# matteosantama/dantzig

Hardware: AMD Instinct MI355X
Metric: simplex_iterations_per_sec (higher is better)
Workload: dtype f64

## Files before the change

dantzig_amd/csrc/k_price.hip:

```cpp
#include "k_price_kernels.h"

static_assert(DZG_RL_WORK_SLOTS == DZG_PRICE_CSC_BLOCKS, "work counters of k_price_csc_rl");

static int resolve(int kernel)
{
    return kernel == DZG_PRICE_WAVE || kernel == DZG_PRICE_TREE ? kernel : DZG_PRICE_SEQ;
}

#define PRICE_ARGS ctl, A, lda, m, q, plist, nonbasis, var_col, v, dz, z, zbar, rz_r, rz_k, rz_h, col0

static void launch_tree(int ncols, const DzgCtl *ctl, const double *A, long long lda, int m, int q,
                        const int *plist, const int *nonbasis, const int *var_col, const double *v,
                        double *dz, const double *z, const double *zbar, double *rz_r, int *rz_k,
                        double *rz_h, int col0, const int *pcode, hipStream_t st, int rows_T = 0,
                        int need_kind = -1)
{
    const dim3 grid(DZG_PRICE_TREE_BLOCKS), block(256);
    const int per_wave = (ncols + 4 * DZG_PRICE_TREE_BLOCKS - 1) / (4 * DZG_PRICE_TREE_BLOCKS);
    const int passes = (per_wave + 15) / 16;
    const int cw = passes > 0 ? (per_wave + passes - 1) / passes : 1;
#define TREE(CW, DEPTH, TP)                                                                          \
    hipLaunchKernelGGL((k_price_tree<CW, DEPTH, TP>), grid, block, 0, st, PRICE_ARGS, pcode, rows_T, need_kind)
    if (per_wave == 15 || per_wave == 16) { TREE(8, 2, 2); return; }
    switch (cw) {
    case 16: TREE(16, 2, 1); break;
    case 15: TREE(15, 2, 1); break;
    case 14: TREE(14, 2, 1); break;
    case 13: TREE(13, 2, 1); break;
    case 12: TREE(12, 3, 1); break;
    case 11: TREE(11, 3, 1); break;
    case 10: TREE(10, 2, 2); break;
    case 9: TREE(9, 2, 2); break;
    case 8: TREE(8, 2, 2); break;
    case 7: TREE(7, 4, 1); break;
    case 6: TREE(6, 3, 2); break;
    case 5: TREE(5, 4, 2); break;
    case 4: TREE(4, 8, 1); break;
    case 3: TREE(3, 10, 1); break;
    case 2: TREE(2, 16, 1); break;
    default: TREE(1, 32, 1); break;
    }
#undef TREE
}

static void launch(int kernel, int ncols, const DzgCtl *ctl, const double *A, long long lda, int m, int q,
                   const int *plist, const int *nonbasis, const int *var_col, const double *v,
                   double *dz, const double *z, const double *zbar, double *rz_r, int *rz_k,
                   double *rz_h, int col0, const int *pcode, hipStream_t st, int rows_T = 0,
                   int need_kind = -1)
{
    if (q <= 0) return;
    if (resolve(kernel) == DZG_PRICE_TREE)
        launch_tree(ncols, PRICE_ARGS, pcode, st, rows_T, need_kind);
    else if (resolve(kernel) == DZG_PRICE_WAVE)
        hipLaunchKernelGGL((k_price_wave2<4>), dim3(DZG_PRICE_WAVE_BLOCKS), dim3(256), 0, st, ctl, A,
                           lda, m, q, plist, nonbasis, var_col, v, dz, z, zbar, rz_r, rz_k, rz_h, col0);
    else
        hipLaunchKernelGGL((k_price_seq2<16>), dim3(DZG_PRICE_SEQ_BLOCKS), dim3(256), 0, st, ctl, A,
                           lda, m, q, plist, nonbasis, var_col, v, dz, z, zbar, rz_r, rz_k, rz_h, col0);
}

int dzg_price_partials(int kernel)
{
    if (kernel == DZG_PRICE_CSC_KERNEL) return DZG_PRICE_CSC_BLOCKS;
    if (resolve(kernel) == DZG_PRICE_TREE) return DZG_PRICE_TREE_BLOCKS;
    return resolve(kernel) == DZG_PRICE_WAVE ? DZG_PRICE_WAVE_BLOCKS : DZG_PRICE_SEQ_BLOCKS;
}

static int rl_grid(void)
{
    static const int g = [] {
        const char *e = std::getenv("DZG_RL_GRID");
        const int v = e ? std::atoi(e) : 1024;
        return v < 1 ? 1 : (v > DZG_PRICE_CSC_BLOCKS ? DZG_PRICE_CSC_BLOCKS : v);
    }();
    return g;
}

int dzg_price_partials_dev(const DzgDev &d, int kernel)
{
    if (!d.csc) return dzg_price_partials(kernel);
    if (d.spb && d.lcnt && kernel != DZG_PRICE_SEQ) return rl_grid();
    return DZG_PRICE_CSC_BLOCKS;
}

static void launch_csc(const DzgDev &d, const int *plist, const double *z, const double *zbar,
                       double *rz_r, int *rz_k, double *rz_h, bool seq_order, hipStream_t st)
{
    if (d.q <= 0) return;
    if (z && !seq_order)
        hipLaunchKernelGGL(k_price_csc_tree, dim3(DZG_PRICE_CSC_BLOCKS), dim3(256), 0, st, d.ctl,
                           d.cptr, d.ridx, d.cval, d.q, plist, d.nbcode, (const int *)nullptr, d.v,
                           d.dz, z, zbar, rz_r, rz_k, rz_h, d.col0, plist ? d.pcode : (const int *)nullptr);
    else
        hipLaunchKernelGGL(k_price_csc, dim3(DZG_PRICE_CSC_BLOCKS), dim3(256), 0, st, d.ctl, d.cptr,
                           d.ridx, d.cval, d.q, plist, d.nonbasis, d.var_col, d.v, d.dz, z, zbar,
                           rz_r, rz_k, rz_h, d.col0);
}

void dzg_launch_price(const DzgDev &d, int kernel, hipStream_t st)
{
    if (d.csc) {
        launch_csc(d, nullptr, nullptr, nullptr, nullptr, nullptr, nullptr, true, st);
        return;
    }
    launch(kernel, d.q, d.ctl, d.A, d.lda, d.m, d.q, nullptr, d.nonbasis, d.var_col, d.v, d.dz, nullptr,
           nullptr, nullptr, nullptr, nullptr, 0, nullptr, st);
}

void dzg_launch_transpose_to_rows(const double *A, long long lda, int m, int n, double *At,
                                  long long ldt, hipStream_t st)
{
    if (m <= 0 || ldt <= 0) return;
    hipLaunchKernelGGL(k_transpose_to_rows, dim3((unsigned)((ldt + 31) / 32), (unsigned)((m + 31) / 32)),
                       dim3(32, 8), 0, st, A, lda, m, n, At, ldt);
}
int dzg_price_rows_groups(void) { return PR_GMAX; }

static int price_small_k(void)
{
    static const int v = [] {
        const char *e = std::getenv("DZG_PRICE_SMALL_K");
        const int x = e ? std::atoi(e) : 480;
        return x < 0 ? 0 : (x > PRS_ROWS - 1 ? PRS_ROWS - 1 : x);
    }();
    return v;
}
int dzg_price_small(const DzgDev &d, int kernel)
{
    return d.cpos && d.vc && d.world <= 1 && !d.rs && dzg_price_rows_certain(d, kernel) && d.k_hint < price_small_k() &&
           (d.ldt + PRS_TILE - 1) / PRS_TILE <= 4096;
}
int dzg_price_small_partials(const DzgDev &d) { return (int)((d.ldt + PRS_TILE - 1) / PRS_TILE); }

int dzg_price_rows_certain(const DzgDev &d, int kernel)
{
    return !d.csc && d.At && d.q > 0 && resolve(kernel) == DZG_PRICE_TREE && d.k_hint > 0 &&
           d.k_hint < d.rows_T && d.k_hint < d.fold_k;
}

void dzg_launch_price_fast(const DzgDev &d, int kernel, hipStream_t st, int need_kind, int skip_finish,
                           int small, unsigned long long *dbg)
{
    if (small) {
        if (d.k_hint < 8 * DZG_PR_BATCH - 1)
            hipLaunchKernelGGL(k_price_rows_small<false>, dim3(dzg_price_small_partials(d)), dim3(512), 0, st,
                               d.ctl, d.rows_T, d.At, d.ldt, d.col1 - d.col0, d.drow, d.vc, d.cpos, d.q,
                               d.nbcode, d.v, d.dz, d.z, d.zbar, d.rz_r, d.rz_k, d.rz_h, dbg);
        else
            hipLaunchKernelGGL(k_price_rows_small<true>, dim3(dzg_price_small_partials(d)), dim3(512), 0, st,
                               d.ctl, d.rows_T, d.At, d.ldt, d.col1 - d.col0, d.drow, d.vc, d.cpos, d.q,
                               d.nbcode, d.v, d.dz, d.z, d.zbar, d.rz_r, d.rz_k, d.rz_h, dbg);
        return;
    }
    if (d.csc) {
        if (d.spb && d.lcnt && kernel != DZG_PRICE_SEQ) {
            if (d.q > 0)
                hipLaunchKernelGGL(k_price_csc_rl, dim3(rl_grid()), dim3(256), 0, st, d.ctl,
                                   d.cptr, d.lcnt, d.lent, d.q, d.plist, d.pcode, d.nbcode, d.v,
                                   d.dz, d.z, d.zbar, d.rz_r, d.rz_k, d.rz_h, d.rl_work);
            return;
        }
        launch_csc(d, d.plist, d.z, d.zbar, d.rz_r, d.rz_k, d.rz_h, kernel == DZG_PRICE_SEQ, st);
        return;
    }
    int ncols = d.col1 - d.col0;
    if (d.price_cols_hint > 0 && d.price_cols_hint < ncols) ncols = d.price_cols_hint;
    int rows_T = 0;
    if (d.At && d.q > 0 && resolve(kernel) == DZG_PRICE_TREE) {
        rows_T = d.rows_T;
        const bool rows_possible = d.k_lo_hint < 0 || d.k_lo_hint < rows_T;
        const bool cols_possible = d.k_hint <= 0 || d.k_hint >= rows_T;
        const int rows_rule = cols_possible ? rows_T : 0x7fffffff;
        if (!rows_possible) rows_T = 0;
        if (rows_possible) {
            hipLaunchKernelGGL((k_price_rows<2>), dim3((unsigned)((d.ldt + 511) / 512), PR_GMAX),
                               dim3(256), 0, st, d.ctl, rows_rule, d.At, d.ldt, d.drow, d.bcode, d.vc,
                               d.ppart, need_kind);
            if (!(skip_finish && !cols_possible))
                hipLaunchKernelGGL(k_price_rows_finish, dim3(DZG_PRICE_TREE_BLOCKS), dim3(256), 0, st,
                                   d.ctl, rows_rule, d.ppart, d.ldt, d.q, d.plist, d.pcode, d.nbcode, d.bcode,
                                   d.col0, d.v, d.dz, d.z, d.zbar, d.rz_r, d.rz_k, d.rz_h, PR_GMAX, need_kind);
        }
        if (!cols_possible) return;
    }
    launch(kernel, ncols, d.ctl, d.A, d.lda, d.m, d.q, d.plist, d.nbcode, nullptr, d.v, d.dz, d.z,
           d.zbar, d.rz_r, d.rz_k, d.rz_h, d.col0, d.pcode, st, rows_T, need_kind);
}

void dzg_launch_price_raw(int kernel, int m, long long lda, const double *A, const int *cols,
                          int ncols, const double *v, double *out, hipStream_t st)
{
    launch(kernel, ncols, nullptr, A, lda, m, ncols, nullptr, cols, nullptr, v, out, nullptr, nullptr,
           nullptr, nullptr, nullptr, 0, nullptr, st);
}

void dzg_launch_price_csc_raw(const long long *cptr, const int *ridx, const double *cval,
                              const int *cols, int ncols, const double *v, double *out,
                              hipStream_t st)
{
    if (ncols <= 0) return;
    hipLaunchKernelGGL(k_price_csc, dim3(DZG_PRICE_CSC_BLOCKS), dim3(256), 0, st,
                       (const DzgCtl *)nullptr, cptr, ridx, cval, ncols, (const int *)nullptr, cols,
                       (const int *)nullptr, v, out, (const double *)nullptr,
                       (const double *)nullptr, (double *)nullptr, (int *)nullptr,
                       (double *)nullptr, 0);
}
```

dantzig_amd/csrc/k_price_kernels.h:

```cpp
#pragma once
#include "common.h"

typedef double double2_t __attribute__((ext_vector_type(2)));

__device__ __forceinline__ int price_code(const int *__restrict__ nonbasis,
                                          const int *__restrict__ var_col, int pos)
{
    const int v = nonbasis[pos];
    return var_col ? var_col[v] : v;
}

__device__ __forceinline__ void price_candidate(DzgCand2 &best, double dzk, int pos, double mu,
                                                double tau, const double *__restrict__ z,
                                                const double *__restrict__ zbar)
{
    const double zk = z[pos], scaled = mu * zbar[pos];
    const double den = zk + scaled;
    DzgCand2 c;
    c.r = dzg_div(dzk, den);
    c.k = pos;
    c.h = -__builtin_inf();
    if (c.r > 0.0) best = dzg_better2(best, c);
    if (dzg_noise_zero(den, zk, scaled, tau)) best.h = __builtin_inf();
}

__device__ __forceinline__ void price_candidate_v(DzgCand2 &best, double dzk, int pos, double mu,
                                                  double tau, double zk, double zbk)
{
    const double scaled = mu * zbk;
    const double den = zk + scaled;
    DzgCand2 c;
    c.r = dzg_div(dzk, den);
    c.k = pos;
    c.h = -__builtin_inf();
    if (c.r > 0.0) best = dzg_better2(best, c);
    if (dzg_noise_zero(den, zk, scaled, tau)) best.h = __builtin_inf();
}

__device__ __forceinline__ void price_slack_positions(DzgCand2 &best, int q,
                                                      const int *__restrict__ nonbasis,
                                                      const int *__restrict__ var_col,
                                                      const double *__restrict__ v,
                                                      double *__restrict__ dz, double mu,
                                                      double tau, const double *__restrict__ z,
                                                      const double *__restrict__ zbar)
{
    const int nthreads = gridDim.x * blockDim.x;
    for (int pos = blockIdx.x * blockDim.x + threadIdx.x; pos < q; pos += nthreads) {
        const int code = price_code(nonbasis, var_col, pos);
        if (code < 0) {
            const double p = 1.0 * -v[-1 - code];
            const double d = 0.0 + p;
            dz[pos] = d;
            if (z) price_candidate(best, d, pos, mu, tau, z, zbar);
        }
    }
}

__device__ __forceinline__ void price_publish(DzgCand2 best, double *__restrict__ rz_r,
                                              int *__restrict__ rz_k, double *__restrict__ rz_h)
{
    best = dzg_block_best2(best);
    if (rz_r && threadIdx.x == 0) {
        rz_r[blockIdx.x] = best.r;
        rz_k[blockIdx.x] = best.k;
        rz_h[blockIdx.x] = best.h;
    }
}

__device__ __forceinline__ void price_publish_small(DzgCand2 best, double *__restrict__ rz_r,
                                                    int *__restrict__ rz_k, double *__restrict__ rz_h)
{
    best = dzg_block_best2_flat<8>(best, false);
    if (rz_r && threadIdx.x == 0) {
        rz_r[blockIdx.x] = best.r;
        rz_k[blockIdx.x] = best.k;
        rz_h[blockIdx.x] = best.h;
    }
}

template <int CW, int DEPTH = 2, int DBG = 0, bool NT = true>
__global__ __launch_bounds__(256) void k_price_seq2(
    const DzgCtl *ctl, const double *__restrict__ A, long long lda, int m, int q,
    const int *__restrict__ plist, const int *__restrict__ nonbasis,
    const int *__restrict__ var_col, const double *__restrict__ v, double *__restrict__ dz,
    const double *__restrict__ z, const double *__restrict__ zbar, double *__restrict__ rz_r,
    int *__restrict__ rz_k, double *__restrict__ rz_h, int col0 = 0)
{
    constexpr int TR = 128, PAD = 2;
    __shared__ __attribute__((aligned(16))) double tile[4][CW][TR + PAD];
    if (ctl && ctl->status != DZG_RUNNING) return;
    const int lane = threadIdx.x & 63, wave = threadIdx.x >> 6;
    const int nw = gridDim.x * 4;
    const int wg = blockIdx.x * 4 + wave;
    const double mu = ctl ? ctl->mu : 0.0, tau = ctl ? ctl->tau : 0.0;
    DzgCand2 best = dzg_cand2_none();
    price_slack_positions(best, q, nonbasis, var_col, v, dz, mu, tau, z, zbar);

    const int count = plist ? (int)ctl->nb_struct : q;
    const int base = count / nw, rem = count % nw;
    const int start = wg * base + (wg < rem ? wg : rem);
    const int cnt = base + (wg < rem ? 1 : 0);
    const int ntiles = (m + TR - 1) / TR;
    double(*mytile)[TR + PAD] = tile[wave];

    for (int c0 = 0; c0 < cnt; c0 += CW) {
        const int nc = (cnt - c0) < CW ? (cnt - c0) : CW;
        int mypos = -1, mycode = -1;
        if (lane < nc) {
            const int idx = start + c0 + lane;
            mypos = plist ? plist[idx] : idx;
            mycode = price_code(nonbasis, var_col, mypos);
        }
        int lastcode = col0;
#pragma unroll
        for (int l = 0; l < CW; ++l) {
            const int code_l = __builtin_amdgcn_readlane(mycode, l);
            if (code_l >= 0) lastcode = code_l;
        }
        long long off[CW];
#pragma unroll
        for (int l = 0; l < CW; ++l) {
            const int code_l = __builtin_amdgcn_readlane(mycode, l);
            off[l] = (long long)((code_l >= 0 ? code_l : lastcode) - col0) * lda;
        }
        double2_t rg[DEPTH][CW], vg[DEPTH];
        double dbg_sink = 0.0;
        long long cyc_park = 0, cyc_fetch = 0, cyc_walk = 0;
        const int lastpair = (int)lda - 2;
        const int lastv = ((m + 1) & ~1) - 2 >= 0 ? ((m + 1) & ~1) - 2 : 0;

        auto fetch = [&](int t, double2_t(&reg)[CW], double2_t &vreg) {
            const int row = t * TR + 2 * lane;
            const int rowc = row < lda ? row : lastpair;
#pragma unroll
            for (int l = 0; l < CW; ++l) {
                const double2_t *gp = reinterpret_cast<const double2_t *>(A + off[l] + rowc);
                reg[l] = NT ? __builtin_nontemporal_load(gp) : *gp;
            }
            vreg = *reinterpret_cast<const double2_t *>(v + (row < m ? row : lastv));
        };
        auto park = [&](int t, const double2_t(&reg)[CW], const double2_t &vreg) {
            if (DBG == 2) {
#pragma unroll
                for (int l = 0; l < CW; ++l) dbg_sink += reg[l].x + reg[l].y;
                return;
            }
            const int row = t * TR + 2 * lane;
            const bool inside = row < lda && row < m + 1;
            const double nv0 = -vreg.x, nv1 = -vreg.y;
            const double2_t zero = {0.0, 0.0};
            __builtin_amdgcn_wave_barrier();
#pragma unroll
            for (int l = 0; l < CW; ++l) {
                double2_t pr;
                pr.x = reg[l].x != 0.0 ? reg[l].x * nv0 : 0.0;
                pr.y = reg[l].y != 0.0 ? reg[l].y * nv1 : 0.0;
                *reinterpret_cast<double2_t *>(&mytile[l][2 * lane]) = inside ? pr : zero;
            }
            __builtin_amdgcn_fence(__ATOMIC_RELEASE, "wavefront");
            __builtin_amdgcn_wave_barrier();
        };
        double acc = 0.0;
        const double *colp = mytile[lane & (CW - 1)];
        auto walk = [&](int t) {
            if (DBG != 0 && DBG != 4) return;
            const int row0 = t * TR;
            const int rows = (m - row0) < TR ? (m - row0) : TR;
            if (lane < CW) {
                if (rows == TR) {
                    double2_t buf[2][8];
#pragma unroll
                    for (int j = 0; j < 8; ++j)
                        buf[0][j] = *reinterpret_cast<const double2_t *>(colp + 2 * j);
#pragma unroll
                    for (int c = 0; c < TR / 16; ++c) {
                        if (c + 1 < TR / 16) {
#pragma unroll
                            for (int j = 0; j < 8; ++j)
                                buf[(c + 1) & 1][j] = *reinterpret_cast<const double2_t *>(
                                    colp + 16 * (c + 1) + 2 * j);
                        }
#pragma unroll
                        for (int j = 0; j < 8; ++j) {
                            acc = acc + buf[c & 1][j].x;
                            acc = acc + buf[c & 1][j].y;
                        }
                    }
                } else {
                    for (int r = 0; r < rows; ++r) acc = acc + colp[r];
                }
            }
        };

#pragma unroll
        for (int d = 0; d < DEPTH; ++d) fetch(d < ntiles ? d : ntiles - 1, rg[d], vg[d]);
        int t = 0;
        for (; t + 2 * DEPTH - 1 < ntiles; t += DEPTH) {
#pragma unroll
            for (int d = 0; d < DEPTH; ++d) {
                if (DBG == 4) {
                    const long long s0 = __builtin_amdgcn_s_memtime();
                    park(t + d, rg[d], vg[d]);
                    __builtin_amdgcn_s_waitcnt(0xC07F);
                    const long long s1 = __builtin_amdgcn_s_memtime();
                    fetch(t + DEPTH + d, rg[d], vg[d]);
                    const long long s2 = __builtin_amdgcn_s_memtime();
                    walk(t + d);
                    asm volatile("" ::"v"(acc));
                    const long long s3 = __builtin_amdgcn_s_memtime();
                    cyc_park += s1 - s0;
                    cyc_fetch += s2 - s1;
                    cyc_walk += s3 - s2;
                } else {
                    park(t + d, rg[d], vg[d]);
                    fetch(t + DEPTH + d, rg[d], vg[d]);
                    walk(t + d);
                }
            }
        }
#pragma unroll
        for (int d = 0; d < DEPTH; ++d) {
            if (t + d < ntiles) {
                park(t + d, rg[d], vg[d]);
                if (t + DEPTH + d < ntiles) fetch(t + DEPTH + d, rg[d], vg[d]);
                walk(t + d);
            }
        }
#pragma unroll
        for (int d = 0; d < DEPTH; ++d) {
            if (t + DEPTH + d < ntiles) {
                park(t + DEPTH + d, rg[d], vg[d]);
                walk(t + DEPTH + d);
            }
        }
        if (DBG != 0 && DBG != 4) acc = dbg_sink + mytile[lane & (CW - 1)][lane];
        if (DBG == 4 && lane == 0) {
            dz[q + 3 * wg + 0] = (double)cyc_park;
            dz[q + 3 * wg + 1] = (double)cyc_fetch;
            dz[q + 3 * wg + 2] = (double)cyc_walk;
        }
        if (lane < nc && mycode >= 0) {
            dz[mypos] = acc;
            if (z) price_candidate(best, acc, mypos, mu, tau, z, zbar);
        }
    }
    price_publish(best, rz_r, rz_k, rz_h);
}

template <int U>
__global__ __launch_bounds__(256) void k_price_wave2(
    const DzgCtl *ctl, const double *__restrict__ A, long long lda, int m, int q,
    const int *__restrict__ plist, const int *__restrict__ nonbasis,
    const int *__restrict__ var_col, const double *__restrict__ v, double *__restrict__ dz,
    const double *__restrict__ z, const double *__restrict__ zbar, double *__restrict__ rz_r,
    int *__restrict__ rz_k, double *__restrict__ rz_h, int col0 = 0)
{
    if (ctl && ctl->status != DZG_RUNNING) return;
    const int lane = threadIdx.x & 63;
    const int wg = (blockIdx.x * blockDim.x + threadIdx.x) >> 6;
    const int nw = (gridDim.x * blockDim.x) >> 6;
    const double mu = ctl ? ctl->mu : 0.0, tau = ctl ? ctl->tau : 0.0;
    DzgCand2 best = dzg_cand2_none();
    price_slack_positions(best, q, nonbasis, var_col, v, dz, mu, tau, z, zbar);
    const int count = plist ? (int)ctl->nb_struct : q;
    const int mpad = (m + 1) & ~1;
    for (int idx = wg; idx < count; idx += nw) {
        const int pos = plist ? plist[idx] : idx;
        const int code = price_code(nonbasis, var_col, pos);
        if (code < 0) continue;
        const double *col = A + (long long)(code - col0) * lda;
        double acc[U];
#pragma unroll
        for (int u = 0; u < U; ++u) acc[u] = 0.0;
        int r = 2 * lane;
        for (; r + 128 * (U - 1) < mpad; r += 128 * U) {
            double2_t c[U], w[U];
#pragma unroll
            for (int u = 0; u < U; ++u)
                c[u] = __builtin_nontemporal_load(
                    reinterpret_cast<const double2_t *>(col + r + 128 * u));
#pragma unroll
            for (int u = 0; u < U; ++u) w[u] = *reinterpret_cast<const double2_t *>(v + r + 128 * u);
#pragma unroll
            for (int u = 0; u < U; ++u) {
                acc[u] = fma(c[u].x, w[u].x, acc[u]);
                acc[u] = fma(c[u].y, w[u].y, acc[u]);
            }
        }
        for (; r < mpad; r += 128) {
            const double2_t c0 = *reinterpret_cast<const double2_t *>(col + r);
            const double2_t w0 = *reinterpret_cast<const double2_t *>(v + r);
            acc[0] = fma(c0.x, w0.x, acc[0]);
            acc[0] = fma(c0.y, w0.y, acc[0]);
        }
        double s = 0.0;
#pragma unroll
        for (int u = 0; u < U; ++u) s += acc[u];
#pragma unroll
        for (int off = 32; off > 0; off >>= 1) s += __shfl_xor(s, off, DZG_WAVE);
        if (lane == 0) {
            dz[pos] = -s;
            if (z) price_candidate(best, -s, pos, mu, tau, z, zbar);
        }
    }
    price_publish(best, rz_r, rz_k, rz_h);
}

template <int CW, int DEPTH, int TP = 1>
__global__ __launch_bounds__(256) void k_price_tree(
    const DzgCtl *ctl, const double *__restrict__ A, long long lda, int m, int q,
    const int *__restrict__ plist, const int *__restrict__ nonbasis,
    const int *__restrict__ var_col, const double *__restrict__ v, double *__restrict__ dz,
    const double *__restrict__ z, const double *__restrict__ zbar, double *__restrict__ rz_r,
    int *__restrict__ rz_k, double *__restrict__ rz_h, int col0 = 0,
    const int *__restrict__ pcode = nullptr, int rows_T = 0, int need_kind = -1)
{
    constexpr int TR = 128;
    if (ctl && ctl->status != DZG_RUNNING) return;
    if (rows_T > 0 && ctl->ncompact < rows_T) return;
    if (need_kind >= 0 && ctl->kind != need_kind) return;
    const int lane = threadIdx.x & 63, wave = threadIdx.x >> 6;
    const int nw = gridDim.x * 4;
    const int wg = blockIdx.x * 4 + wave;
    const double mu = ctl ? ctl->mu : 0.0, tau = ctl ? ctl->tau : 0.0;
    DzgCand2 best = dzg_cand2_none();
    const int nthreads = gridDim.x * blockDim.x;
    const int spos = blockIdx.x * blockDim.x + threadIdx.x;
    int scode = 0;
    if (spos < q) scode = price_code(nonbasis, var_col, spos);
    double sv = 0.0, sz = 0.0, szb = 0.0;
    bool slack_loaded = false;

    const int count = plist ? (int)ctl->nb_struct : q;
    const int base = count / nw, rem = count % nw;
    const int start = wg * base + (wg < rem ? wg : rem);
    const int cnt = base + (wg < rem ? 1 : 0);
    const int ntiles = (m + TR - 1) / TR;
    const int ngroups = (ntiles + TP - 1) / TP;
    const int lastpair = (int)lda - 2;
    const int lastv = ((m + 1) & ~1) - 2 >= 0 ? ((m + 1) & ~1) - 2 : 0;

    for (int c0 = 0; c0 < cnt; c0 += CW) {
        const int nc = (cnt - c0) < CW ? (cnt - c0) : CW;
        int mypos = -1, mycode = -1;
        if (lane < nc) {
            const int idx = start + c0 + lane;
            mypos = plist ? plist[idx] : idx;
            mycode = pcode ? pcode[idx] : price_code(nonbasis, var_col, mypos);
        }
        int lastcode = col0;
#pragma unroll
        for (int l = 0; l < CW; ++l) {
            const int code_l = __builtin_amdgcn_readlane(mycode, l);
            if (code_l >= 0) lastcode = code_l;
        }
        long long off[CW];
#pragma unroll
        for (int l = 0; l < CW; ++l) {
            const int code_l = __builtin_amdgcn_readlane(mycode, l);
            off[l] = (long long)((code_l >= 0 ? code_l : lastcode) - col0) * lda;
        }
        double2_t rg[DEPTH][TP][CW], vg[DEPTH][TP];
        double acc[CW];
#pragma unroll
        for (int l = 0; l < CW; ++l) acc[l] = 0.0;
        double zc = 0.0, zbc = 0.0;
        if (z && lane < nc && mycode >= 0) {
            zc = z[mypos];
            zbc = zbar[mypos];
        }
        if (!slack_loaded) {
            slack_loaded = true;
            if (scode < 0) {
                sv = v[-1 - scode];
                if (z) {
                    sz = z[spos];
                    szb = zbar[spos];
                }
            }
        }

        auto fetch = [&](int g, double2_t(&reg)[TP][CW], double2_t(&vreg)[TP]) {
#pragma unroll
            for (int l = 0; l < CW; ++l)
#pragma unroll
                for (int u = 0; u < TP; ++u) {
                    const int row = (g * TP + u) * TR + 2 * lane;
                    const int rowc = row < lda ? row : lastpair;
                    reg[u][l] = __builtin_nontemporal_load(
                        reinterpret_cast<const double2_t *>(A + off[l] + rowc));
                }
#pragma unroll
            for (int u = 0; u < TP; ++u) {
                const int row = (g * TP + u) * TR + 2 * lane;
                vreg[u] = *reinterpret_cast<const double2_t *>(v + (row < m ? row : lastv));
            }
        };
        auto consume = [&](int g, const double2_t(&reg)[TP][CW], const double2_t(&vreg)[TP]) {
#pragma unroll
            for (int u = 0; u < TP; ++u) {
                const bool inside = (g * TP + u) * TR + 2 * lane < m;
#pragma unroll
                for (int l = 0; l < CW; ++l) {
                    const double ax = inside ? reg[u][l].x : 0.0, ay = inside ? reg[u][l].y : 0.0;
                    acc[l] = fma(ax, vreg[u].x, acc[l]);
                    acc[l] = fma(ay, vreg[u].y, acc[l]);
                }
            }
        };
#pragma unroll
        for (int d = 0; d < DEPTH; ++d) fetch(d < ngroups ? d : ngroups - 1, rg[d], vg[d]);
        int t = 0;
        for (; t + 2 * DEPTH - 1 < ngroups; t += DEPTH) {
#pragma unroll
            for (int d = 0; d < DEPTH; ++d) {
                consume(t + d, rg[d], vg[d]);
                fetch(t + DEPTH + d, rg[d], vg[d]);
            }
        }
#pragma unroll
        for (int d = 0; d < DEPTH; ++d) {
            if (t + d < ngroups) {
                consume(t + d, rg[d], vg[d]);
                if (t + DEPTH + d < ngroups) fetch(t + DEPTH + d, rg[d], vg[d]);
            }
        }
#pragma unroll
        for (int d = 0; d < DEPTH; ++d)
            if (t + DEPTH + d < ngroups) consume(t + DEPTH + d, rg[d], vg[d]);
        double mine = 0.0;
#pragma unroll
        for (int l = 0; l < CW; ++l) {
            double s = acc[l];
#pragma unroll
            for (int o = 32; o > 0; o >>= 1) s += __shfl_xor(s, o, DZG_WAVE);
            if (lane == l) mine = s;
        }
        if (lane < nc && mycode >= 0) {
            dz[mypos] = -mine;
            if (z) price_candidate_v(best, -mine, mypos, mu, tau, zc, zbc);
        }
    }
    if (scode < 0) {
        if (!slack_loaded) {
            sv = v[-1 - scode];
            if (z) {
                sz = z[spos];
                szb = zbar[spos];
            }
        }
        const double p = 1.0 * -sv;
        const double d = 0.0 + p;
        dz[spos] = d;
        if (z) price_candidate_v(best, d, spos, mu, tau, sz, szb);
    }
    for (int pos = spos + nthreads; pos < q; pos += nthreads) {
        const int code = price_code(nonbasis, var_col, pos);
        if (code < 0) {
            const double p = 1.0 * -v[-1 - code];
            const double d = 0.0 + p;
            dz[pos] = d;
            if (z) price_candidate(best, d, pos, mu, tau, z, zbar);
        }
    }
    price_publish(best, rz_r, rz_k, rz_h);
}

__global__ __launch_bounds__(256) void k_price_csc(
    const DzgCtl *ctl, const long long *__restrict__ cptr, const int *__restrict__ ridx,
    const double *__restrict__ cval, int q, const int *__restrict__ plist,
    const int *__restrict__ nonbasis, const int *__restrict__ var_col,
    const double *__restrict__ v, double *__restrict__ dz, const double *__restrict__ z,
    const double *__restrict__ zbar, double *__restrict__ rz_r, int *__restrict__ rz_k,
    double *__restrict__ rz_h, int col0)
{
    if (ctl && ctl->status != DZG_RUNNING) return;
    const double mu = ctl ? ctl->mu : 0.0, tau = ctl ? ctl->tau : 0.0;
    DzgCand2 best = dzg_cand2_none();
    price_slack_positions(best, q, nonbasis, var_col, v, dz, mu, tau, z, zbar);
    const int count = plist ? (int)ctl->nb_struct : q;
    const int lane = threadIdx.x & 63, sub = lane & 7, gbase = lane & ~7;
    const int group = (blockIdx.x * blockDim.x + threadIdx.x) >> 3;
    const int ngroups = (gridDim.x * blockDim.x) >> 3;
    for (int idx0 = 0; idx0 < count; idx0 += ngroups) {
        const int idx = idx0 + group;
        int pos = -1, code = -1;
        long long e0 = 0, e1 = 0;
        if (idx < count) {
            pos = plist ? plist[idx] : idx;
            code = price_code(nonbasis, var_col, pos);
            if (code >= 0) {
                e0 = cptr[code - col0];
                e1 = cptr[code - col0 + 1];
            }
        }
        long long span = e1 - e0;
#pragma unroll
        for (int off = 32; off >= 8; off >>= 1) {
            const long long o = __shfl_xor(span, off, DZG_WAVE);
            span = o > span ? o : span;
        }
        double acc = 0.0;
        for (long long base = 0; base < span; base += 8) {
            const long long e = e0 + base + sub;
            double p = 0.0;
            if (e < e1) p = cval[e] * -v[ridx[e]];
#pragma unroll
            for (int t = 0; t < 8; ++t) {
                const double pt = __shfl(p, gbase + t, DZG_WAVE);
                if (e0 + base + t < e1) acc = acc + pt;
            }
        }
        if (code >= 0 && sub == 0) {
            dz[pos] = acc;
            if (z) price_candidate(best, acc, pos, mu, tau, z, zbar);
        }
    }
    price_publish(best, rz_r, rz_k, rz_h);
}

__global__ __launch_bounds__(256) void k_price_csc_tree(
    const DzgCtl *ctl, const long long *__restrict__ cptr, const int *__restrict__ ridx,
    const double *__restrict__ cval, int q, const int *__restrict__ plist,
    const int *__restrict__ nonbasis, const int *__restrict__ var_col,
    const double *__restrict__ v, double *__restrict__ dz, const double *__restrict__ z,
    const double *__restrict__ zbar, double *__restrict__ rz_r, int *__restrict__ rz_k,
    double *__restrict__ rz_h, int col0, const int *__restrict__ pcode = nullptr)
{
    if (ctl && ctl->status != DZG_RUNNING) return;
    const double mu = ctl ? ctl->mu : 0.0, tau = ctl ? ctl->tau : 0.0;
    DzgCand2 best = dzg_cand2_none();
    const int nthreads = gridDim.x * blockDim.x;
    const int spos = blockIdx.x * blockDim.x + threadIdx.x;
    int scode = 0;
    if (spos < q) scode = price_code(nonbasis, var_col, spos);
    double sv = 0.0, sz = 0.0, szb = 0.0;
    bool slack_loaded = false;
    const int count = plist ? (int)ctl->nb_struct : q;
    const int sub = threadIdx.x & 7;
    const int group = (blockIdx.x * blockDim.x + threadIdx.x) >> 3;
    const int ngroups = (gridDim.x * blockDim.x) >> 3;
    for (int idx0 = 0; idx0 < count; idx0 += ngroups) {
        const int idx = idx0 + group;
        int pos = -1, code = -1;
        long long e0 = 0, e1 = 0;
        if (idx < count) {
            pos = plist ? plist[idx] : idx;
            code = pcode ? pcode[idx] : price_code(nonbasis, var_col, pos);
            if (code >= 0) {
                e0 = cptr[code - col0];
                e1 = cptr[code - col0 + 1];
            }
        }
        double zc = 0.0, zbc = 0.0;
        if (z && code >= 0 && sub == 0) {
            zc = z[pos];
            zbc = zbar[pos];
        }
        if (!slack_loaded) {
            slack_loaded = true;
            if (scode < 0) {
                sv = v[-1 - scode];
                if (z) {
                    sz = z[spos];
                    szb = zbar[spos];
                }
            }
        }
        double a0 = 0.0, a1 = 0.0;
        long long e = e0 + sub;
        for (; e + 8 < e1; e += 16) {
            const int r0 = ridx[e], r1 = ridx[e + 8];
            const double c0 = cval[e], c1 = cval[e + 8];
            a0 = fma(c0, v[r0], a0);
            a1 = fma(c1, v[r1], a1);
        }
        if (e < e1) a0 = fma(cval[e], v[ridx[e]], a0);
        double acc = a0 + a1;
#pragma unroll
        for (int off = 4; off > 0; off >>= 1) acc += __shfl_xor(acc, off, DZG_WAVE);
        if (code >= 0 && sub == 0) {
            dz[pos] = -acc;
            if (z) price_candidate_v(best, -acc, pos, mu, tau, zc, zbc);
        }
    }
    if (scode < 0) {
        if (!slack_loaded) {
            sv = v[-1 - scode];
            if (z) {
                sz = z[spos];
                szb = zbar[spos];
            }
        }
        const double p = 1.0 * -sv;
        const double d = 0.0 + p;
        dz[spos] = d;
        if (z) price_candidate_v(best, d, spos, mu, tau, sz, szb);
    }
    for (int pos = spos + nthreads; pos < q; pos += nthreads) {
        const int code = price_code(nonbasis, var_col, pos);
        if (code < 0) {
            const double p = 1.0 * -v[-1 - code];
            const double d = 0.0 + p;
            dz[pos] = d;
            if (z) price_candidate(best, d, pos, mu, tau, z, zbar);
        }
    }
    price_publish(best, rz_r, rz_k, rz_h);
}

#define RL_LPC 4
__global__ __launch_bounds__(256) void k_price_csc_rl(
    const DzgCtl *ctl, const long long *__restrict__ cptr, const int *__restrict__ lcnt,
    const DzgLiveEntry *__restrict__ lent, int q,
    const int *__restrict__ plist, const int *__restrict__ pcode, const int *__restrict__ nbcode,
    const double *__restrict__ v, double *__restrict__ dz, const double *__restrict__ z,
    const double *__restrict__ zbar, double *__restrict__ rz_r, int *__restrict__ rz_k,
    double *__restrict__ rz_h, unsigned long long *__restrict__ work)
{
    __shared__ unsigned int s_work[4];
    const int nthreads = gridDim.x * blockDim.x;
    const int spos = blockIdx.x * blockDim.x + threadIdx.x;
    const int sub = threadIdx.x & (RL_LPC - 1);
    const int group = spos / RL_LPC;
    const int ngroups = nthreads / RL_LPC;
    int scode = 0, pos0 = -1, code0 = -1;
    if (spos < q) scode = nbcode[spos];
    if (group < q) {
        pos0 = plist[group];
        code0 = pcode[group];
    }
    const int status = ctl->status, count = (int)ctl->nb_struct;
    const double mu = ctl->mu, tau = ctl->tau;
    if (status != DZG_RUNNING) return;
    DzgCand2 best = dzg_cand2_none();
    double sv = 0.0, sz = 0.0, szb = 0.0;
    if (scode < 0) {
        sv = v[-1 - scode];
        sz = z[spos];
        szb = zbar[spos];
    }
    unsigned int walked = 0;
    for (int idx0 = 0; idx0 < count; idx0 += ngroups) {
        const int idx = idx0 + group;
        int pos = -1, code = -1;
        long long e0 = 0, e1 = 0;
        if (idx < count) {
            pos = idx0 == 0 ? pos0 : plist[idx];
            code = idx0 == 0 ? code0 : pcode[idx];
            if (code >= 0) {
                e0 = cptr[code];
                e1 = e0 + lcnt[code];
            }
        }
        double zc = 0.0, zbc = 0.0;
        if (code >= 0 && sub == 0) {
            zc = z[pos];
            zbc = zbar[pos];
            walked += (unsigned int)(e1 - e0);
        }
        double a0 = 0.0, a1 = 0.0;
        long long e = e0 + sub;
        for (; e + RL_LPC < e1; e += 2 * RL_LPC) {
            const DzgLiveEntry n0 = lent[e], n1 = lent[e + RL_LPC];
            a0 = fma(n0.val, v[n0.row], a0);
            a1 = fma(n1.val, v[n1.row], a1);
        }
        if (e < e1) {
            const DzgLiveEntry n0 = lent[e];
            a0 = fma(n0.val, v[n0.row], a0);
        }
        double acc = a0 + a1;
#pragma unroll
        for (int off = RL_LPC / 2; off > 0; off >>= 1) acc += __shfl_xor(acc, off, DZG_WAVE);
        if (code >= 0 && sub == 0) {
            dz[pos] = -acc;
            price_candidate_v(best, -acc, pos, mu, tau, zc, zbc);
        }
    }
    if (scode < 0) {
        const double p = 1.0 * -sv;
        const double d = 0.0 + p;
        dz[spos] = d;
        price_candidate_v(best, d, spos, mu, tau, sz, szb);
    }
    for (int pos = spos + nthreads; pos < q; pos += nthreads) {
        const int code = nbcode[pos];
        if (code < 0) {
            const double p = 1.0 * -v[-1 - code];
            const double d = 0.0 + p;
            dz[pos] = d;
            price_candidate(best, d, pos, mu, tau, z, zbar);
        }
    }
#pragma unroll
    for (int off = 32; off > 0; off >>= 1) walked += __shfl_xor(walked, off, DZG_WAVE);
    if ((threadIdx.x & 63) == 0) s_work[threadIdx.x >> 6] = walked;
    price_publish(best, rz_r, rz_k, rz_h);
    if (threadIdx.x == 0)
        __hip_atomic_fetch_add(work + blockIdx.x,
                               (unsigned long long)s_work[0] + s_work[1] + s_work[2] + s_work[3],
                               __ATOMIC_RELAXED, __HIP_MEMORY_SCOPE_AGENT);
}

#define PR_GMAX DZG_PR_GMAX
#define PR_BATCH DZG_PR_BATCH
#define PR_PIPE 8
template <int VEC, int PIPE = PR_PIPE>
__global__ __launch_bounds__(256) void k_price_rows(
    const DzgCtl *ctl, int rows_T, const double *__restrict__ At, long long ldt,
    const int *__restrict__ drow, const int *__restrict__ bcode, const double *__restrict__ vc,
    double *__restrict__ part, int need_kind = -1)
{
    typedef double vec_t __attribute__((ext_vector_type(2)));
    __shared__ long long s_off[256];
    __shared__ double s_coef[256];
    const int status = ctl->status, k = ctl->ncompact, lp = ctl->leave_pos;
    if (status != DZG_RUNNING || k >= rows_T) return;
    if (need_kind >= 0 && ctl->kind != need_kind) return;
    int G = (k + 1 + PR_BATCH - 1) / PR_BATCH;
    G = G > (int)gridDim.y ? (int)gridDim.y : G;
    const int g = blockIdx.y;
    if (g >= G) return;
    const int lcode = lp >= 0 ? bcode[lp] : 0;
    const int nrows = k + (lcode < 0 ? 1 : 0);
    const long long j0 = ((long long)blockIdx.x * 256 + threadIdx.x) * VEC;
    const bool live = j0 < ldt;
    const double *col = At + (live ? j0 : 0);
    double acc[VEC];
#pragma unroll
    for (int e = 0; e < VEC; ++e) acc[e] = 0.0;
    for (int cbase = g; cbase < nrows; cbase += 256 * G) {
        __syncthreads();
        const int c = cbase + (int)threadIdx.x * G;
        if (c < nrows) {
            const int row = c < k ? drow[c] : -1 - lcode;
            s_off[threadIdx.x] = (long long)row * ldt;
            s_coef[threadIdx.x] = c < k ? vc[c] : 1.0;
        }
        __syncthreads();
        const int left = (nrows - cbase + G - 1) / G;
        const int n = left < 256 ? left : 256;
        const int bfull = n / PIPE;
        vec_t ra[PIPE][VEC / 2], rb[PIPE][VEC / 2];
#define PR_LOAD(B, REG)                                                                              \
    _Pragma("unroll") for (int u = 0; u < PIPE; ++u) {                                            \
        const double *src = col + s_off[(B) * PIPE + u];                                          \
        _Pragma("unroll") for (int h = 0; h < VEC / 2; ++h)                                          \
            REG[u][h] = __builtin_nontemporal_load(reinterpret_cast<const vec_t *>(src) + h);        \
    }
#define PR_FMA(B, REG)                                                                               \
    _Pragma("unroll") for (int u = 0; u < PIPE; ++u) {                                            \
        const double cf = s_coef[(B) * PIPE + u];                                                 \
        _Pragma("unroll") for (int h = 0; h < VEC / 2; ++h) {                                        \
            acc[2 * h] = fma(cf, REG[u][h].x, acc[2 * h]);                                           \
            acc[2 * h + 1] = fma(cf, REG[u][h].y, acc[2 * h + 1]);                                   \
        }                                                                                            \
    }
        int bi = 0;
        if (bfull > 0) { PR_LOAD(0, ra) }
        while (bi + 2 < bfull) {
            PR_LOAD(bi + 1, rb)
            PR_FMA(bi, ra)
            PR_LOAD(bi + 2, ra)
            PR_FMA(bi + 1, rb)
            bi += 2;
        }
        if (bfull - bi == 2) {
            PR_LOAD(bi + 1, rb)
            PR_FMA(bi, ra)
            PR_FMA(bi + 1, rb)
        } else if (bfull - bi == 1) {
            PR_FMA(bi, ra)
        }
#undef PR_LOAD
#undef PR_FMA
        {
            const int i0 = bfull * PIPE;
#pragma unroll
            for (int u = 0; u < PIPE; ++u)
                if (i0 + u < n) {
                    const double *src = col + s_off[i0 + u];
#pragma unroll
                    for (int h = 0; h < VEC / 2; ++h)
                        ra[u][h] = __builtin_nontemporal_load(reinterpret_cast<const vec_t *>(src) + h);
                }
#pragma unroll
            for (int u = 0; u < PIPE; ++u)
                if (i0 + u < n) {
                    const double cf = s_coef[i0 + u];
#pragma unroll
                    for (int h = 0; h < VEC / 2; ++h) {
                        acc[2 * h] = fma(cf, ra[u][h].x, acc[2 * h]);
                        acc[2 * h + 1] = fma(cf, ra[u][h].y, acc[2 * h + 1]);
                    }
                }
        }
    }
    if (live) {
        double *dst = part + (long long)g * ldt + j0;
#pragma unroll
        for (int e = 0; e < VEC; ++e) dst[e] = acc[e];
    }
}

#define PRS_TILE 64
#define PRS_ROWS 512
#define PRS_STAMP_SLOT 4
template <bool WIDE>
__global__ __launch_bounds__(512) void k_price_rows_small(
    const DzgCtl *__restrict__ ctl, int rows_T, const double *__restrict__ At, long long ldt, int ncols,
    const int *__restrict__ drow, const double *__restrict__ vc,
    const int *__restrict__ cpos, int q, const int *__restrict__ nbcode, const double *__restrict__ v,
    double *__restrict__ dz, const double *__restrict__ z, const double *__restrict__ zbar,
    double *__restrict__ rz_r, int *__restrict__ rz_k, double *__restrict__ rz_h,
    unsigned long long *dbg)
{
    __shared__ long long s_off[PRS_ROWS];
    __shared__ double s_coef[PRS_ROWS];
    __shared__ double s_part[PR_GMAX][PRS_TILE];
    ChainStamps ts;
    ts.start(dbg);
    const int tid = threadIdx.x, lane = tid & 63, wave = tid >> 6;
    const int spos = blockIdx.x * 512 + tid;
    int scode = 0;
    if (spos < q) scode = nbcode[spos];
    const long long j = (long long)blockIdx.x * PRS_TILE + lane;
    int pos = -1;
    if (wave == 0 && j < ncols) pos = cpos[j];
    const int status = ctl->status, k = ctl->ncompact, lp = ctl->leave_pos;
    const int lcode_c = ctl->leave_code;
    const double mu = ctl->mu, tau = ctl->tau;
    asm volatile("" ::"s"(status), "s"(k), "s"(lp), "s"(lcode_c), "s"(mu), "s"(tau));
    if (status != DZG_RUNNING || k >= rows_T || k >= PRS_ROWS) return;
    ts.mark(PRS_STAMP_SLOT);
    const int lcode = lp >= 0 ? lcode_c : 0;
    if (tid < k) {
        s_off[tid] = (long long)drow[tid] * ldt;
        s_coef[tid] = vc[tid];
    }
    double sv = 0.0, sz = 0.0, szb = 0.0, zc = 0.0, zbc = 0.0;
    if (scode < 0) {
        sv = v[-1 - scode];
        sz = z[spos];
        szb = zbar[spos];
    }
    if (pos >= 0) {
        zc = z[pos];
        zbc = zbar[pos];
    }
    const int nrows = k + (lcode < 0 ? 1 : 0);
    if (tid == k && lcode < 0) {
        s_off[k] = (long long)(-1 - lcode) * ldt;
        s_coef[k] = 1.0;
    }
    int G = (k + 1 + PR_BATCH - 1) / PR_BATCH;
    G = G > PR_GMAX ? PR_GMAX : G;
    __syncthreads();
    ts.mark(PRS_STAMP_SLOT);
    const double *col = At + (j < ldt ? j : 0);
    if (WIDE) {
        double acc[4] = {0.0, 0.0, 0.0, 0.0};
        const int rpg = (nrows + G - 1) / G;
        for (int r0 = 0; r0 < rpg; r0 += 8) {
            double vv[4][8];
#pragma unroll
            for (int t = 0; t < 4; ++t) {
                const int g = wave + 8 * t;
#pragma unroll
                for (int u = 0; u < 8; ++u) {
                    const int c = g + (r0 + u) * G;
                    vv[t][u] = (g < G && c < nrows) ? __builtin_nontemporal_load(col + s_off[c]) : 0.0;
                }
            }
#pragma unroll
            for (int t = 0; t < 4; ++t) {
                const int g = wave + 8 * t;
#pragma unroll
                for (int u = 0; u < 8; ++u) {
                    const int c = g + (r0 + u) * G;
                    if (g < G && c < nrows) acc[t] = fma(s_coef[c], vv[t][u], acc[t]);
                }
            }
        }
#pragma unroll
        for (int t = 0; t < 4; ++t)
            if (wave + 8 * t < G) s_part[wave + 8 * t][lane] = acc[t];
    } else {
        for (int g = wave; g < G; g += 8) {
            double acc = 0.0;
            for (int c0 = g; c0 < nrows; c0 += 8 * G) {
                double vv[8];
#pragma unroll
                for (int u = 0; u < 8; ++u) {
                    const int c = c0 + u * G;
                    vv[u] = c < nrows ? __builtin_nontemporal_load(col + s_off[c]) : 0.0;
                }
#pragma unroll
                for (int u = 0; u < 8; ++u) {
                    const int c = c0 + u * G;
                    if (c < nrows) acc = fma(s_coef[c], vv[u], acc);
                }
            }
            s_part[g][lane] = acc;
        }
    }
    __syncthreads();
    ts.mark(PRS_STAMP_SLOT);
    DzgCand2 best = dzg_cand2_none();
    if (pos >= 0) {
        double sum = 0.0;
        for (int g = 0; g < G; ++g) sum = sum + s_part[g][lane];
        dz[pos] = -sum;
        price_candidate_v(best, -sum, pos, mu, tau, zc, zbc);
    }
    if (scode < 0) {
        const double p = 1.0 * -sv;
        const double d = 0.0 + p;
        dz[spos] = d;
        price_candidate_v(best, d, spos, mu, tau, sz, szb);
    }
    for (int ps = spos + (int)gridDim.x * 512; ps < q; ps += (int)gridDim.x * 512) {
        const int code = nbcode[ps];
        if (code < 0) {
            const double p = 1.0 * -v[-1 - code];
            const double d = 0.0 + p;
            dz[ps] = d;
            price_candidate(best, d, ps, mu, tau, z, zbar);
        }
    }
    ts.pin(best);
    const unsigned long long t_publish = ts.now();
    price_publish_small(best, rz_r, rz_k, rz_h);
    ts.site(DZG_SITE_PUBLISH, t_publish);
    ts.mark(PRS_STAMP_SLOT);
    ts.done(PRS_STAMP_SLOT);
}

__global__ __launch_bounds__(256) void k_price_rows_finish(
    const DzgCtl *ctl, int rows_T, const double *__restrict__ part, long long ldt, int q,
    const int *__restrict__ plist, const int *__restrict__ pcode, const int *__restrict__ nbcode,
    const int *__restrict__ bcode, int col0, const double *__restrict__ v, double *__restrict__ dz,
    const double *__restrict__ z, const double *__restrict__ zbar, double *__restrict__ rz_r,
    int *__restrict__ rz_k, double *__restrict__ rz_h, int gmax, int need_kind = -1)
{
    const int nthreads = gridDim.x * blockDim.x;
    const int spos = blockIdx.x * blockDim.x + threadIdx.x;
    int scode = 0, pos0 = -1, code0 = -1;
    if (spos < q) {
        scode = nbcode[spos];
        pos0 = plist[spos];
        code0 = pcode[spos];
    }
    const int status = ctl->status, k = ctl->ncompact;
    const int count = (int)ctl->nb_struct;
    const double mu = ctl->mu, tau = ctl->tau;
    if (status != DZG_RUNNING || k >= rows_T) return;
    if (need_kind >= 0 && ctl->kind != need_kind) return;
    int G = (k + 1 + PR_BATCH - 1) / PR_BATCH;
    G = G > gmax ? gmax : G;
    DzgCand2 best = dzg_cand2_none();
    double sv = 0.0, sz = 0.0, szb = 0.0;
    if (scode < 0) {
        sv = v[-1 - scode];
        sz = z[spos];
        szb = zbar[spos];
    }
    for (int idx = spos; idx < count; idx += nthreads) {
        const int pos = idx == spos ? pos0 : plist[idx];
        const int code = idx == spos ? code0 : pcode[idx];
        if (code < 0) continue;
        const double zc = z[pos], zbc = zbar[pos];
        const double *src = part + (code - col0);
        double sum = 0.0;
        int gg = 0;
        for (; gg + 8 <= G; gg += 8) {
            double t[8];
#pragma unroll
            for (int e = 0; e < 8; ++e) t[e] = src[(long long)(gg + e) * ldt];
#pragma unroll
            for (int e = 0; e < 8; ++e) sum = sum + t[e];
        }
        for (; gg < G; ++gg) sum = sum + src[(long long)gg * ldt];
        dz[pos] = -sum;
        price_candidate_v(best, -sum, pos, mu, tau, zc, zbc);
    }
    if (scode < 0) {
        const double p = 1.0 * -sv;
        const double d = 0.0 + p;
        dz[spos] = d;
        price_candidate_v(best, d, spos, mu, tau, sz, szb);
    }
    for (int pos = spos + nthreads; pos < q; pos += nthreads) {
        const int code = nbcode[pos];
        if (code < 0) {
            const double p = 1.0 * -v[-1 - code];
            const double d = 0.0 + p;
            dz[pos] = d;
            price_candidate(best, d, pos, mu, tau, z, zbar);
        }
    }
    price_publish(best, rz_r, rz_k, rz_h);
}

__global__ __launch_bounds__(256) void k_transpose_to_rows(const double *__restrict__ A, long long lda,
                                                           int m, int n, double *__restrict__ At,
                                                           long long ldt)
{
    __shared__ double tile[32][33];
    const int j0 = blockIdx.x * 32, i0 = blockIdx.y * 32;
    for (int jj = threadIdx.y; jj < 32; jj += 8) {
        const int j = j0 + jj, i = i0 + threadIdx.x;
        tile[jj][threadIdx.x] = (j < n && i < m) ? A[(long long)j * lda + i] : 0.0;
    }
    __syncthreads();
    for (int ii = threadIdx.y; ii < 32; ii += 8) {
        const int i = i0 + ii, j = j0 + threadIdx.x;
        if (i < m && j < ldt) At[(long long)i * ldt + j] = tile[threadIdx.x][ii];
    }
}

#define DZG_PRICE_CSC_BLOCKS 2048
#define DZG_PRICE_SEQ_BLOCKS 256
#define DZG_PRICE_WAVE_BLOCKS 2048
#define DZG_PRICE_TREE_BLOCKS 256
```

Baseline: 33730.

## Generalize small-k row pricing kernel with vector loads and tunable group tiling

```diff
diff --git a/dantzig_amd/csrc/k_price.hip b/dantzig_amd/csrc/k_price.hip
--- a/dantzig_amd/csrc/k_price.hip
+++ b/dantzig_amd/csrc/k_price.hip
@@ -126,10 +126,22 @@
     }();
     return v;
 }
+static int price_cus(void)
+{
+    static const int v = [] {
+        int dev = 0, n = 0;
+        if (hipGetDevice(&dev) != hipSuccess ||
+            hipDeviceGetAttribute(&n, hipDeviceAttributeMultiprocessorCount, dev) != hipSuccess || n < 1)
+            n = 256;
+        return n;
+    }();
+    return v;
+}
 int dzg_price_small(const DzgDev &d, int kernel)
 {
+    const bool aligned = (d.ldt & 1) == 0 && (reinterpret_cast<uintptr_t>(d.At) & 15) == 0;
     return d.cpos && d.vc && d.world <= 1 && !d.rs && dzg_price_rows_certain(d, kernel) && d.k_hint < price_small_k() &&
-           (d.ldt + PRS_TILE - 1) / PRS_TILE <= 4096;
+           (d.ldt + PRS_TILE - 1) / PRS_TILE <= 4096 && aligned;
 }
 int dzg_price_small_partials(const DzgDev &d) { return (int)((d.ldt + PRS_TILE - 1) / PRS_TILE); }
 
@@ -143,14 +155,18 @@
                            int small, unsigned long long *dbg)
 {
     if (small) {
-        if (d.k_hint < 8 * DZG_PR_BATCH - 1)
-            hipLaunchKernelGGL(k_price_rows_small<false>, dim3(dzg_price_small_partials(d)), dim3(512), 0, st,
-                               d.ctl, d.rows_T, d.At, d.ldt, d.col1 - d.col0, d.drow, d.vc, d.cpos, d.q,
-                               d.nbcode, d.v, d.dz, d.z, d.zbar, d.rz_r, d.rz_k, d.rz_h, dbg);
+        const int tiles = dzg_price_small_partials(d);
+#define SMALL(VEC, NG, RPT)                                                                          \
+    hipLaunchKernelGGL((k_price_rows_small<VEC, NG, RPT>), dim3(tiles), dim3(512), 0, st, d.ctl, d.rows_T, \
+                       d.At, d.ldt, d.col1 - d.col0, d.drow, d.vc, d.m, d.cpos, d.q, d.nbcode, d.v, d.dz, d.z, \
+                       d.zbar, d.rz_r, d.rz_k, d.rz_h, dbg)
+        if (d.k_hint < 8 * DZG_PR_BATCH - 1 && tiles > 2 * price_cus())
+            SMALL(1, 1, 8);
+        else if (d.k_hint < 16 * DZG_PR_BATCH - 1)
+            SMALL(2, 1, 16);
         else
-            hipLaunchKernelGGL(k_price_rows_small<true>, dim3(dzg_price_small_partials(d)), dim3(512), 0, st,
-                               d.ctl, d.rows_T, d.At, d.ldt, d.col1 - d.col0, d.drow, d.vc, d.cpos, d.q,
-                               d.nbcode, d.v, d.dz, d.z, d.zbar, d.rz_r, d.rz_k, d.rz_h, dbg);
+            SMALL(2, 2, 16);
+#undef SMALL
         return;
     }
     if (d.csc) {
diff --git a/dantzig_amd/csrc/k_price_kernels.h b/dantzig_amd/csrc/k_price_kernels.h
--- a/dantzig_amd/csrc/k_price_kernels.h
+++ b/dantzig_amd/csrc/k_price_kernels.h
@@ -808,18 +808,22 @@
 #define PRS_TILE 64
 #define PRS_ROWS 512
 #define PRS_STAMP_SLOT 4
-template <bool WIDE>
-__global__ __launch_bounds__(512) void k_price_rows_small(
-    const DzgCtl *__restrict__ ctl, int rows_T, const double *__restrict__ At, long long ldt, int ncols,
-    const int *__restrict__ drow, const double *__restrict__ vc,
+template <int VEC, int NG, int RPT>
+__global__ __launch_bounds__(512, (RPT < PR_BATCH ? 8 : 2)) void k_price_rows_small(
+    DzgCtl *__restrict__ ctl, int rows_T, const double *__restrict__ At, long long ldt, int ncols,
+    const int *__restrict__ drow, const double *__restrict__ vc, int m,
     const int *__restrict__ cpos, int q, const int *__restrict__ nbcode, const double *__restrict__ v,
     double *__restrict__ dz, const double *__restrict__ z, const double *__restrict__ zbar,
     double *__restrict__ rz_r, int *__restrict__ rz_k, double *__restrict__ rz_h,
     unsigned long long *dbg)
 {
+    constexpr int LPG = 64 / VEC;
+    constexpr int NS = 512 / LPG;
+    static_assert(VEC == 1 || VEC == 2, "8- or 16-byte loads");
+    static_assert(PR_BATCH % RPT == 0 && PR_GMAX * PR_BATCH >= PRS_ROWS, "a group has at most PR_BATCH rows");
     __shared__ long long s_off[PRS_ROWS];
     __shared__ double s_coef[PRS_ROWS];
-    __shared__ double s_part[PR_GMAX][PRS_TILE];
+    __shared__ __attribute__((aligned(16))) double s_part[PR_GMAX][PRS_TILE];
     ChainStamps ts;
     ts.start(dbg);
     const int tid = threadIdx.x, lane = tid & 63, wave = tid >> 6;
@@ -829,17 +833,27 @@
     const long long j = (long long)blockIdx.x * PRS_TILE + lane;
     int pos = -1;
     if (wave == 0 && j < ncols) pos = cpos[j];
+    const int li = tid < m ? tid : m - 1;
+    const int lrow = drow[li];
+    const double lcf = vc[li];
     const int status = ctl->status, k = ctl->ncompact, lp = ctl->leave_pos;
     const int lcode_c = ctl->leave_code;
     const double mu = ctl->mu, tau = ctl->tau;
     asm volatile("" ::"s"(status), "s"(k), "s"(lp), "s"(lcode_c), "s"(mu), "s"(tau));
-    if (status != DZG_RUNNING || k >= rows_T || k >= PRS_ROWS) return;
+    if (status != DZG_RUNNING) return;
+    if (k >= rows_T || k >= PRS_ROWS) {
+        if (blockIdx.x == 0 && tid == 0) ctl->status = DZG_PANIC;
+        return;
+    }
     ts.mark(PRS_STAMP_SLOT);
     const int lcode = lp >= 0 ? lcode_c : 0;
-    if (tid < k) {
-        s_off[tid] = (long long)drow[tid] * ldt;
-        s_coef[tid] = vc[tid];
-    }
+    {
+        const bool own = tid == k && lcode < 0;
+        s_off[tid] = (long long)(own ? -1 - lcode : lrow) * ldt;
+        s_coef[tid] = own ? 1.0 : lcf;
+    }
+    __syncthreads();
+    ts.mark(PRS_STAMP_SLOT);
     double sv = 0.0, sz = 0.0, szb = 0.0, zc = 0.0, zbc = 0.0;
     if (scode < 0) {
         sv = v[-1 - scode];
@@ -851,60 +865,70 @@
         zbc = zbar[pos];
     }
     const int nrows = k + (lcode < 0 ? 1 : 0);
-    if (tid == k && lcode < 0) {
-        s_off[k] = (long long)(-1 - lcode) * ldt;
-        s_coef[k] = 1.0;
-    }
     int G = (k + 1 + PR_BATCH - 1) / PR_BATCH;
     G = G > PR_GMAX ? PR_GMAX : G;
-    __syncthreads();
-    ts.mark(PRS_STAMP_SLOT);
-    const double *col = At + (j < ldt ? j : 0);
-    if (WIDE) {
-        double acc[4] = {0.0, 0.0, 0.0, 0.0};
-        const int rpg = (nrows + G - 1) / G;
-        for (int r0 = 0; r0 < rpg; r0 += 8) {
-            double vv[4][8];
-#pragma unroll
-            for (int t = 0; t < 4; ++t) {
-                const int g = wave + 8 * t;
-#pragma unroll
-                for (int u = 0; u < 8; ++u) {
-                    const int c = g + (r0 + u) * G;
-                    vv[t][u] = (g < G && c < nrows) ? __builtin_nontemporal_load(col + s_off[c]) : 0.0;
-                }
-            }
-#pragma unroll
-            for (int t = 0; t < 4; ++t) {
-                const int g = wave + 8 * t;
-#pragma unroll
-                for (int u = 0; u < 8; ++u) {
-                    const int c = g + (r0 + u) * G;
-                    if (g < G && c < nrows) acc[t] = fma(s_coef[c], vv[t][u], acc[t]);
-                }
-            }
-        }
-#pragma unroll
-        for (int t = 0; t < 4; ++t)
-            if (wave + 8 * t < G) s_part[wave + 8 * t][lane] = acc[t];
-    } else {
-        for (int g = wave; g < G; g += 8) {
-            double acc = 0.0;
-            for (int c0 = g; c0 < nrows; c0 += 8 * G) {
-                double vv[8];
-#pragma unroll
-                for (int u = 0; u < 8; ++u) {
-                    const int c = c0 + u * G;
-                    vv[u] = c < nrows ? __builtin_nontemporal_load(col + s_off[c]) : 0.0;
-                }
-#pragma unroll
-                for (int u = 0; u < 8; ++u) {
-                    const int c = c0 + u * G;
-                    if (c < nrows) acc = fma(s_coef[c], vv[u], acc);
-                }
-            }
-            s_part[g][lane] = acc;
-        }
+    const int slot = tid / LPG, h = tid % LPG;
+    const long long jc = (long long)blockIdx.x * PRS_TILE + h * VEC;
+    const double *col = At + (jc < ldt ? jc : 0);
+    for (int g0 = slot; g0 < G; g0 += NS * NG) {
+        double acc[NG][VEC];
+#pragma unroll
+        for (int t = 0; t < NG; ++t)
+#pragma unroll
+            for (int e = 0; e < VEC; ++e) acc[t][e] = 0.0;
+        for (int r0 = 0; r0 < PR_BATCH; r0 += RPT) {
+            if (RPT < PR_BATCH && g0 + r0 * G >= nrows) break;
+#define PRS_ENTRY(T, U)                                                                              \
+    const int c = g0 + NS * (T) + (r0 + (U)) * G;                                                    \
+    const bool ok = g0 + NS * (T) < G && c < nrows
+            long long off[NG][RPT];
+#pragma unroll
+            for (int t = 0; t < NG; ++t)
+#pragma unroll
+                for (int u = 0; u < RPT; ++u) {
+                    PRS_ENTRY(t, u);
+                    off[t][u] = s_off[ok ? c : 0];
+                }
+            double x[NG][RPT][VEC], cf[NG][RPT];
+#pragma unroll
+            for (int t = 0; t < NG; ++t)
+#pragma unroll
+                for (int u = 0; u < RPT; ++u) {
+                    PRS_ENTRY(t, u);
+                    const double *src = col + (ok ? off[t][u] : 0);
+                    if constexpr (VEC == 2) {
+                        const double2_t w = __builtin_nontemporal_load(reinterpret_cast<const double2_t *>(src));
+                        x[t][u][0] = w.x;
+                        x[t][u][1] = w.y;
+                    } else {
+                        x[t][u][0] = __builtin_nontemporal_load(src);
+                    }
+                }
+            __builtin_amdgcn_sched_barrier(0);
+#pragma unroll
+            for (int t = 0; t < NG; ++t)
+#pragma unroll
+                for (int u = 0; u < RPT; ++u) {
+                    PRS_ENTRY(t, u);
+                    cf[t][u] = s_coef[ok ? c : 0];
+                }
+#pragma unroll
+            for (int t = 0; t < NG; ++t)
+#pragma unroll
+                for (int u = 0; u < RPT; ++u) {
+                    PRS_ENTRY(t, u);
+#pragma unroll
+                    for (int e = 0; e < VEC; ++e)
+                        acc[t][e] = ok ? fma(cf[t][u], x[t][u][e], acc[t][e]) : acc[t][e];
+                }
+#undef PRS_ENTRY
+        }
+#pragma unroll
+        for (int t = 0; t < NG; ++t)
+            if (g0 + NS * t < G) {
+#pragma unroll
+                for (int e = 0; e < VEC; ++e) s_part[g0 + NS * t][h * VEC + e] = acc[t][e];
+            }
     }
     __syncthreads();
     ts.mark(PRS_STAMP_SLOT);
```

New measurement: 34220, median of 6. +1.5%, better.
